# qbxlvnf11/yolo-series

Measured on AMD Instinct MI355X. Metric: images/sec (640×640) + mAP@0.5 parity vs ref; 1/2/4/8 MI355X, higher is better.
Workload: dtype f16; 1 GPU; yolov7 P5 640x640 bs=32/GPU f16: libyv7 forward + GPU NMS (conf 0.25, iou 0.45, max_det 300); global_batch=32, img=640, parallelism=dp1, rccl_world_size=1, weights=seeded synthetic, resident_input_batches=4

## Files before the change

yolo-series_amd/csrc/conv_det.hip:

```cpp
#include <cstdlib>

#include "conv_det.h"
#include "conv_f16_launch.h"

namespace yv7 {

namespace {

template <int HOOK = 0>
__global__ __launch_bounds__(512, 1) void conv_det_pring_kernel(const ConvParams p) {
  constexpr int BM = 64, BN = 256, WM = 2, WN = 4, NW = 8, NTH = 512;
  constexpr int WTM = BM / WM, WTN = BN / WN, TM = WTM / 16, TN = WTN / 16;
  constexpr int RB = BN / 8 / NW;
  constexpr int PER = HOOK == 4 ? 1 : 1 + RB;
  constexpr int STAGE = (BM + BN) * ROWB;
  constexpr int RING = 2 * STAGE;
  constexpr int LDS = RING + det_lds(BM, BN);
  static_assert(LDS <= 160 * 1024, "LDS budget");
  __shared__ __attribute__((aligned(16))) unsigned char smem[LDS];
  unsigned char* es = smem + RING;

  const int tid = threadIdx.x, lane = tid & 63;
  const int wave = __builtin_amdgcn_readfirstlane(tid >> 6);
  const int wm = wave / WN, wn = wave % WN;
// ... 4 lines not shown
  const int ntl = tw.count();
  if (ntl == 0) return;

  const auto xr = make_rsrc(p.x, p.xbytes);
  const auto wr = make_rsrc(p.w, p.wbytes);
  const int lr = lane >> 3;
  const int c = (lane & 7) ^ lr;
  uint32_t b_off[RB];
#pragma unroll
  for (int j = 0; j < RB; ++j) b_off[j] = (uint32_t)((((j * NW + wave) * 8 + lr) * p.kpad + c * 8) * 2);
  const int hw = p.Ho * p.Wo;
  auto a_off = [&](int it) -> uint32_t {
    if (it >= ntl) return OOB;
    const int m = tw.at(it) * BM + wave * 8 + lr;
    if (m >= p.M) return OOB;
    const int b = m / hw, cell = m - b * hw, ho = cell / p.Wo, wo = cell - ho * p.Wo;
    return (uint32_t)((pix_index(b, ho, wo, p.H, p.W) * p.xc + p.xoff + c * 8) * 2);
  };
  int i_it = 0, i_k = 0, i_q = 0;
  uint32_t i_aoff = a_off(0);
  auto issue = [&]() __attribute__((always_inline)) {
    unsigned char* As = smem + (i_q & 1) * STAGE;
    unsigned char* Bs = As + BM * ROWB;
    const bool live = i_it < ntl;
    const uint32_t so = (uint32_t)i_k * BKE * 2;
    dma16(xr, As + wave * 8 * ROWB, i_aoff, so);
    if constexpr (HOOK != 4) {
#pragma unroll
      for (int j = 0; j < RB; ++j) dma16(wr, Bs + (j * NW + wave) * 8 * ROWB, live ? b_off[j] : OOB, so);
    }
// ... 121 lines not shown
  const int g = lane >> 4, li = lane & 15;
  const int m0 = blockIdx.x * BM;
  if (m0 >= p.M) return;
  const int nk = p.kpad / BKE;
  const auto xr = make_rsrc(p.x, p.xbytes);
  const auto wr = make_rsrc(p.w, p.wbytes);
  const int lr = lane >> 3;
  const int c = (lane & 7) ^ lr;
  uint32_t b_off[RB];
#pragma unroll
  for (int j = 0; j < RB; ++j) b_off[j] = (uint32_t)((((j * NW + wave) * 8 + lr) * p.kpad + c * 8) * 2);
  const int hw = p.Ho * p.Wo;
  uint32_t aoff = OOB;
  {
    const int m = m0 + wave * 8 + lr;
    if (m < p.M) {
      const int b = m / hw, cell = m - b * hw, ho = cell / p.Wo, wo = cell - ho * p.Wo;
      aoff = (uint32_t)((pix_index(b, ho, wo, p.H, p.W) * p.xc + p.xoff + c * 8) * 2);
    }
  }
  auto issue = [&](int k, int slot) __attribute__((always_inline)) {
    unsigned char* As = smem + slot * STAGE;
    unsigned char* Bs = As + BM * ROWB;
    const uint32_t so = (uint32_t)k * BKE * 2;
    dma16(xr, As + wave * 8 * ROWB, aoff, so);
#pragma unroll
    for (int j = 0; j < RB; ++j) dma16(wr, Bs + (j * NW + wave) * 8 * ROWB, b_off[j], so);
    asm volatile("" ::: "memory");
  };
  f4 acc[TN][TM];
#pragma unroll
// ... 98 lines not shown
  u4 wreg[TN][NCH];
#pragma unroll
  for (int j = 0; j < TN; ++j) {
    const uint32_t base = (uint32_t)(((2 * wave + j) * NCH) * 1024 + lane * 16);
#pragma unroll
    for (int c = 0; c < NCH; ++c)
      wreg[j][c] = __builtin_bit_cast(u4, __builtin_amdgcn_raw_buffer_load_b128(wr, base, (uint32_t)(c * 1024), 0));
  }
  const int lr = lane >> 3;
  const int c8 = (lane & 7) ^ lr;
  const int hw = p.Ho * p.Wo;
  auto a_off = [&](int it) -> uint32_t {
    if (it >= ntl) return OOB;
    const int m = tw.at(it) * BM + (wave % (BM / 8)) * 8 + lr;
    if (m >= p.M) return OOB;
    const int b = m / hw, cell = m - b * hw, ho = cell / p.Wo, wo = cell - ho * p.Wo;
    return (uint32_t)((pix_index(b, ho, wo, p.H, p.W) * p.xc + p.xoff + c8 * 8) * 2);
  };
  int i_it = 0, i_k = 0, i_slot = 0;
  uint32_t i_aoff = a_off(0);
  auto issue = [&]() __attribute__((always_inline)) {
    if constexpr (HOOK != 1) dma16(xr, smem + i_slot * STAGE + (wave % (BM / 8)) * 8 * ROWB, i_aoff, (uint32_t)i_k * BKE * 2);
    asm volatile("" ::: "memory");
    if (++i_slot == R) i_slot = 0;
    if (++i_k == NK) {
      i_k = 0;
      ++i_it;
      i_aoff = a_off(i_it);
    }
  };
// ... 93 lines not shown
}

bool det_rw_supported(const ConvParams& p) {
  return p.wf && (p.kpad == 256 || p.kpad == 512) && p.wfbytes >= (uint32_t)(256 * p.kpad * 2);
}

}

bool det_pring_supported(const ConvParams& p) {
  const int hw = p.Ho * p.Wo;
  return p.k == 1 && p.s == 1 && p.na == 3 && p.no == 85 && p.cout == 255 && p.raw == nullptr &&
         p.kpad == p.cin && p.cin % BKE == 0 && p.cin >= 2 * BKE && hw % 4 == 0 && p.row_off % 4 == 0 &&
         p.nrows % 4 == 0 && p.xoff % 8 == 0 && p.xc % 8 == 0 && p.H == p.Ho && p.W == p.Wo;
}

hipError_t launch_det_pring(const ConvParams& p, hipStream_t st) {
  const long T = (p.M + 63) / 64, cus = device_cus();
  const long per = (T + cus - 1) / cus;
  const int grid = (int)((T + per - 1) / per);
  static const int rw = env_int("YV7_DET_RW", 1);
  if (rw && (p.variant == 0 || p.variant == 91) && det_rw_supported(p)) {
    if (p.variant == 91) {
      if (p.kpad == 256) YV7_LAUNCH((conv_det_rw_kernel<8, 1>), dim3(grid), dim3(512), 0, st, p);
      else YV7_LAUNCH((conv_det_rw_kernel<16, 1>), dim3(grid), dim3(512), 0, st, p);
      return hipGetLastError();
    }
    static const int rwd = env_int("YV7_DET_RWD", 4);
    static const int bm_env = env_int("YV7_DET_BM", 0);
    const int bm = bm_env ? bm_env : (p.kpad == 512 ? 32 : 64);
    if (bm == 32 && rwd == 4) {
      const long T2 = (p.M + 31) / 32, per2 = (T2 + cus - 1) / cus;
// ... 29 lines not shown
```

yolo-series_amd/csrc/conv_f16_common.h:

```cpp
#pragma once
#include "yv7_kernels.h"

namespace yv7 {

namespace {

constexpr int NT = 256;
constexpr int BKE = 64;
constexpr int ROWB = 128;

__device__ __forceinline__ int swz(int row, int chunk) { return chunk ^ (row & 7); }

struct PixelWalk {
  int b, ho, wo;
  __device__ __forceinline__ PixelWalk(const ConvParams& p, int m) {
    const int hw = p.Ho * p.Wo;
    b = m / hw;
    const int rem = m - b * hw;
    ho = rem / p.Wo;
    wo = rem - ho * p.Wo;
  }
  __device__ __forceinline__ void advance(const ConvParams& p, int step) {
    wo += step;
    while (wo >= p.Wo) {
      wo -= p.Wo;
      if (++ho == p.Ho) { ho = 0; ++b; }
    }
  }
};

__device__ __forceinline__ uint32_t a_origin(const ConvParams& p, int b, int ho, int wo, int chunk) {
  return (uint32_t)((pix_index(b, ho * p.s - p.pad, wo * p.s - p.pad, p.H, p.W) * p.xc + p.xoff + chunk * 8) * 2);
}

template <int BK = BKE>
struct KCursor {
  int ci, rr, ss, tap;
  __device__ __forceinline__ void init(const ConvParams& p, int k) {
    ci = k; rr = ss = tap = 0;
    while (ci >= p.cin) { ci -= p.cin; ++tap; if (++ss == p.k) { ss = 0; ++rr; } }
  }
  __device__ __forceinline__ void advance(const ConvParams& p) {
    ci += BK;
    while (ci >= p.cin) { ci -= p.cin; ++tap; if (++ss == p.k) { ss = 0; ++rr; } }
  }
  __device__ __forceinline__ uint32_t offset(const ConvParams& p) const {
    return (uint32_t)(((rr * (p.W + 2 * BORDER) + ss) * p.xc + ci) * 2);
// ... 84 lines not shown
```

yolo-series_amd/csrc/conv_f16_p8.hip:

```cpp
#include "conv_f16_common.h"
#include "conv_f16_launch.h"

namespace yv7 {

namespace {

template <bool ONE, int ACT, int BM = 256, int BN = 256>
__global__ __launch_bounds__(512, 1) void conv_f16_p8_kernel(const ConvParams p) {
  constexpr int NTH = 512;
  constexpr int AHR = BM / 2, BHR = BN / 2;
  constexpr int AHB = AHR * ROWB, BHB = BHR * ROWB;
  constexpr int BUF = 2 * AHB + 2 * BHB;
  constexpr int AP = AHR / 64, BP = BHR / 64;
  constexpr int VMC = 2 * AP + BP;
  constexpr int WNC = BHR / 32;
  static_assert(AP >= 1 && BP >= 1 && (AHR / 64) * WNC == 8, "8 waves of 64 x 32 per block quadrant");
  constexpr int BIASB = (2 * BUF + 4096 + 16 <= 163840) ? 4096 : 0;
  __shared__ __attribute__((aligned(16))) unsigned char smem[2 * BUF + BIASB];
  float* bias_l = reinterpret_cast<float*>(smem + 2 * BUF);

  const int tid = threadIdx.x, lane = tid & 63;
  const int wave = __builtin_amdgcn_readfirstlane(tid >> 6);
  const int wm = wave / WNC, wn = wave % WNC;
  const int grp = wave >> 2;
// ... 11 lines not shown
  auto tile_at = [&](int it) { return tw.at(it); };

  const auto xr = make_rsrc(p.x, p.xbytes);
  const auto wr = make_rsrc(p.w, p.wbytes);
  const auto yr = make_rsrc(p.y, 0x7fffffffu);
  if constexpr (BIASB != 0)
    for (int i = tid; i < p.cout; i += NTH) bias_l[i] = p.bias[i];

  int a_it = 0, a_kt = 0, b_it = 0, b_kt = 0;
  uint32_t a_off[2][AP], b_off[2][BP], a_so = 0;
  KWalk sa, sb;
  auto stage_a = [&](int h, int par) {
    if (h == 0) {
      if (a_kt == 0) {
        const int t = tile_at(a_it);
        PixelWalk pw(p, (t / nN) * BM + wave * 8 + lr);
#pragma unroll
        for (int q = 0; q < 2 * AP; ++q) {
          if (q) pw.advance(p, 64);
          a_off[q / AP][q % AP] = a_origin(p, pw.b, pw.ho, pw.wo, c);
        }
        sa.init();
      }
      a_so = ONE ? (uint32_t)a_kt * BKE * 2 : sa.a_offset(p);
      if (!ONE) sa.advance(p);
    }
    unsigned char* d = smem + par * BUF + h * AHB;
#pragma unroll
    for (int j = 0; j < AP; ++j) dma16(xr, d + (j * 8 + wave) * 8 * ROWB, a_off[h][j], a_so);
    if (h == 1) {
      if (++a_kt == nk) { a_kt = 0; ++a_it; }
    }
  };
  uint32_t b_so = 0;
  auto stage_b = [&](int h, int par) {
    if (h == 1) {
// ... 29 lines not shown
        const int col = cn0 + hb * BHR + wn * 32 + j * 16 + g * 4;
        f4 bv;
#pragma unroll
        for (int e = 0; e < 4; ++e)
          bv[e] = col + e < p.cout ? (BIASB ? bias_l[col + e] : p.bias[col + e]) : 0.0f;
#pragma unroll
        for (int ha = 0; ha < 2; ++ha)
#pragma unroll
          for (int i = 0; i < 4; ++i) acc[hb][j][ha][i] = bv;
      }
  };
  const uint32_t lane_ch = (uint32_t)(16 * (g & 1) + 8 * (g >> 1));
  auto epilogue = [&]() {
#pragma unroll
    for (int ha = 0; ha < 2; ++ha) {
      PixelWalk pw(p, cm0 + ha * AHR + wm * 64 + li);
#pragma unroll
      for (int i = 0; i < 4; ++i) {
        if (i) pw.advance(p, 16);
        const int m = cm0 + ha * AHR + wm * 64 + i * 16 + li;
        const uint32_t yo = (uint32_t)((pix_index(pw.b, pw.ho, pw.wo, p.Ho, p.Wo) * p.yc + p.yoff) * 2);
#pragma unroll
        for (int hb = 0; hb < 2; ++hb) {
          typedef _Float16 h4 __attribute__((ext_vector_type(4)));
          typedef uint32_t u2 __attribute__((ext_vector_type(2)));
          h4 va, vb;
          const f4 a0 = acc[hb][0][ha][i], a1 = acc[hb][1][ha][i];
#pragma unroll
          for (int e = 0; e < 4; ++e) {
            va[e] = (_Float16)act_t<ACT>(a0[e]);
            vb[e] = (_Float16)act_t<ACT>(a1[e]);
          }
          const u2 a = __builtin_bit_cast(u2, va), b = __builtin_bit_cast(u2, vb);
          const auto s0 = __builtin_amdgcn_permlane16_swap(a[0], b[0], false, false);
          const auto s1 = __builtin_amdgcn_permlane16_swap(a[1], b[1], false, false);
          const u4 v = {s0[0], s1[0], s0[1], s1[1]};
// ... 65 lines not shown
    if (n2) stage_a(0, P);
    mfma_q(0, 1);
    read_a(bk + AHB);
    if (n2) stage_b(1, P);
    mfma_q(1, 1);
    read_b(bk + 2 * AHB);
    if (n2) {
      stage_a(1, P);
      asm volatile("s_waitcnt vmcnt(%0)" ::"n"(VMC) : "memory");
    } else {
      asm volatile("s_waitcnt vmcnt(0)" ::: "memory");
    }
    mfma_q(1, 0);
  };
  auto fresh_a = [&](int t) __attribute__((always_inline)) {
    PixelWalk pw(p, (t / nN) * BM + wave * 8 + lr);
#pragma unroll
    for (int q = 0; q < 2 * AP; ++q) {
      if (q) pw.advance(p, 64);
      a_off[q / AP][q % AP] = a_origin(p, pw.b, pw.ho, pw.wo, c);
    }
  };
  auto fresh_b = [&](int t) __attribute__((always_inline)) {
    const int n0 = t % nN * BN;
#pragma unroll
    for (int q = 0; q < 2 * BP; ++q)
      b_off[q / BP][q % BP] = (uint32_t)(((n0 + (q / BP) * BHR + ((q % BP) * 8 + wave) * 8 + lr) * p.kpad + c * 8) * 2);
  };
  auto dma_a = [&](int h, int par, uint32_t so) __attribute__((always_inline)) {
    unsigned char* d = smem + par * BUF + h * AHB;
#pragma unroll
    for (int j = 0; j < AP; ++j) dma16(xr, d + (j * 8 + wave) * 8 * ROWB, a_off[h][j], so);
  };
  auto dma_b = [&](int h, int par, uint32_t so) __attribute__((always_inline)) {
    unsigned char* d = smem + par * BUF + 2 * AHB + h * BHB;
#pragma unroll
// ... 99 lines not shown
  const int total = ntl * nk;
  if (total == 0) return;

  const auto xr = make_rsrc(p.x, p.xbytes);
  const auto wr = make_rsrc(p.w, p.wbytes);
  const auto yr = make_rsrc(p.y, 0x7fffffffu);
  for (int i = tid; i < p.cout; i += NTH) bias_l[i] = p.bias[i];

  int s_it = 0, s_kt = 0;
  uint32_t a_off[2][2], b_off[2], a_so = 0, b_so = 0;
  KWalk su;
  auto stage = [&](int h, int par) {
    if (h == 0) {
      if (s_kt == 0) {
        const int t = tw.at(s_it);
        PixelWalk pw(p, (t / nN) * BM + wave * 8 + lr);
#pragma unroll
        for (int q = 0; q < 4; ++q) {
          if (q) pw.advance(p, 64);
          a_off[q >> 1][q & 1] = a_origin(p, pw.b, pw.ho, pw.wo, c);
        }
        const int n0 = t % nN * BN;
#pragma unroll
        for (int q = 0; q < 2; ++q) b_off[q] = (uint32_t)(((n0 + q * 64 + wave * 8 + lr) * p.kpad + c * 8) * 2);
        su.init();
      }
      a_so = ONE ? (uint32_t)s_kt * BKE * 2 : su.a_offset(p);
      b_so = ONE ? (uint32_t)s_kt * BKE * 2 : su.b_offset(p);
      if (!ONE) su.advance(p);
    }
    unsigned char* d = smem + par * BUF;
#pragma unroll
    for (int j = 0; j < 2; ++j) dma16(xr, d + h * AH + (j * 8 + wave) * 8 * ROWB, a_off[h][j], a_so);
    dma16(wr, d + 2 * AH + h * BH + wave * 8 * ROWB, b_off[h], b_so);
    if (h == 1) {
      if (++s_kt == nk) { s_kt = 0; ++s_it; }
// ... 10 lines not shown
    for (int j = 0; j < 4; ++j) {
      const int col = cn0 + wn * 64 + j * 16 + g * 4;
      f4 bv;
#pragma unroll
      for (int e = 0; e < 4; ++e) bv[e] = col + e < p.cout ? bias_l[col + e] : 0.0f;
#pragma unroll
      for (int h = 0; h < 2; ++h)
#pragma unroll
        for (int i = 0; i < 2; ++i) acc[h][j][i] = bv;
    }
  };
  const uint32_t lane_ch = (uint32_t)(16 * (g & 1) + 8 * (g >> 1));
  auto epilogue = [&]() {
#pragma unroll
    for (int h = 0; h < 2; ++h) {
      PixelWalk pw(p, cm0 + h * 128 + wm * 32 + li);
#pragma unroll
      for (int i = 0; i < 2; ++i) {
        if (i) pw.advance(p, 16);
        const int m = cm0 + h * 128 + wm * 32 + i * 16 + li;
        const uint32_t yo = (uint32_t)((pix_index(pw.b, pw.ho, pw.wo, p.Ho, p.Wo) * p.yc + p.yoff) * 2);
#pragma unroll
        for (int mp = 0; mp < 2; ++mp) {
          typedef _Float16 h4 __attribute__((ext_vector_type(4)));
          typedef uint32_t u2 __attribute__((ext_vector_type(2)));
          h4 va, vb;
#pragma unroll
          for (int e = 0; e < 4; ++e) {
            va[e] = (_Float16)act_t<ACT>(acc[h][2 * mp][i][e]);
            vb[e] = (_Float16)act_t<ACT>(acc[h][2 * mp + 1][i][e]);
          }
          const u2 a = __builtin_bit_cast(u2, va), b = __builtin_bit_cast(u2, vb);
          const auto s0 = __builtin_amdgcn_permlane16_swap(a[0], b[0], false, false);
          const auto s1 = __builtin_amdgcn_permlane16_swap(a[1], b[1], false, false);
          const u4 v = {s0[0], s1[0], s0[1], s1[1]};
          const int n = cn0 + wn * 64 + mp * 32 + (int)lane_ch;
// ... 82 lines not shown
    for (int k = 0; k < total; ++k) {
      ktile(k % 3, k + 2 < total);
      if (++ckt == nk) {
        epilogue();
        ckt = 0;
        if (++ci < ntl) init_tile(ci);
      }
    }
  }
  if (grp == 0) __builtin_amdgcn_s_barrier();
  asm volatile("s_waitcnt vmcnt(0)" ::: "memory");
}

}

hipError_t launch_p8(const ConvParams& p, int cfg, hipStream_t st) {
  const bool one = p.k == 1 && p.s == 1 && p.pad == 0;
  if (cfg != P8_256x256 && cfg != P8_256x128) return hipErrorInvalidValue;
  if (p.cout > 1024 || p.cout % 8 || p.yoff % 8 || p.yc % 8 || (!one && p.cin % BKE)) return hipErrorInvalidValue;
  const int bn = cfg == P8_256x256 ? 256 : 128;
  const long T = (long)((p.M + 255) / 256) * ((p.cout + bn - 1) / bn);
  const int cus = device_cus();
  const int grid = (int)(T < (long)cus ? T : (long)cus);
  return launch_with_act(p.act, [&](auto A) {
    constexpr int ACT = decltype(A)::value;
    if (cfg == P8_256x256) {
      if (one) YV7_LAUNCH((conv_f16_p8_kernel<true, ACT>), dim3(grid), dim3(512), 0, st, p);
      else YV7_LAUNCH((conv_f16_p8_kernel<false, ACT>), dim3(grid), dim3(512), 0, st, p);
    } else {
      if (one) YV7_LAUNCH((conv_f16_p8n_kernel<true, ACT>), dim3(grid), dim3(512), 0, st, p);
      else YV7_LAUNCH((conv_f16_p8n_kernel<false, ACT>), dim3(grid), dim3(512), 0, st, p);
// ... 7 lines not shown
```

yolo-series_amd/csrc/conv_f16_pring.hip:

```cpp
#include "conv_f16_common.h"
#include "conv_f16_launch.h"

namespace yv7 {

namespace {

template <int BM, int BN, int WM, int WN, int STAGES, bool ONE, int ACT, int BK, int WS = 0, int HOOK = 0>
__global__ __launch_bounds__(64 * WM * WN, (STAGES * (BM + BN) * BK * 2 <= 48 * 1024 && WM * WN == 4) ? 3 : (STAGES * (BM + BN) * BK * 2 <= 76 * 1024) ? 2 : 1) void conv_f16_pring_kernel(
    const ConvParams p) {
  constexpr int NW = WM * WN, NTH = 64 * NW;
  constexpr int WTM = BM / WM, WTN = BN / WN;
  constexpr int TM = WTM / 16, TN = WTN / 16;
  constexpr int RB_ = BK * 2;
  constexpr int CPR = RB_ / 16;
  constexpr int RPI = 64 / CPR;
  constexpr int RA = BM / RPI / NW, RB = BN / RPI / NW;
  static_assert(RA * RPI * NW == BM && RB * RPI * NW == BN, "tile rows must split into DMA groups per wave");
  static_assert(TN % 2 == 0, "the epilogue pairs 16-channel groups");
  static_assert(STAGES >= 2 && STAGES <= 4, "counted waits cover up to two stages in flight");
  static_assert(WS == 0 || ONE, "weight-stationary form: 1x1 convs only");
  constexpr int PER = RA + (WS ? 0 : RB);
  constexpr int NST = TM * TN / 2;
  constexpr int STAGE = (BM + (WS ? 0 : BN)) * RB_;
  constexpr int WREG = WS ? BN * WS * RB_ : 0;
// ... 41 lines not shown
    for (int q = wave; q < nk * GPS; q += NW) {
      const int ks = q / GPS, rg = q - ks * GPS;
      dma16(wr, wl + (ks * BN + rg * RPI) * RB_, (uint32_t)(((nb * BN + rg * RPI + lr) * p.kpad + c * 8) * 2),
            (uint32_t)ks * BK * 2);
    }
  }

  AWalk<ONE, RA, BK> aw;
  uint32_t b_off[RB];
  int ig = 0, it = 0, ikt = 0;
  auto issue_next = [&]() __attribute__((always_inline)) {
    if (ikt == 0) {
      const int t = tw.at(it);
      const int m0 = tile_m0(t), n0 = tile_n0(t);
      aw.init(p, c, 0);
      PixelWalk pw(p, m0 + wave * RPI + lr);
#pragma unroll
      for (int j = 0; j < RA; ++j) {
        if (j) pw.advance(p, NW * RPI);
        aw.off[j] = a_origin(p, pw.b, pw.ho, pw.wo, c);
      }
#pragma unroll
      for (int j = 0; j < RB; ++j) b_off[j] = (uint32_t)(((n0 + (j * NW + wave) * RPI + lr) * p.kpad + c * 8) * 2);
    }
    const int slot = ig % STAGES;
    unsigned char* As = smem + slot * STAGE;
    unsigned char* Bs = As + BM * RB_;
    if constexpr (HOOK != 298) {
      aw.step(p, ikt, [&](int j, uint32_t vo, uint32_t so) { dma16(xr, As + (j * NW + wave) * RPI * RB_, vo, so); });
      if constexpr (WS == 0) {
#pragma unroll
        for (int j = 0; j < RB; ++j) dma16(wr, Bs + (j * NW + wave) * RPI * RB_, b_off[j], (uint32_t)ikt * BK * 2);
      }
    }
    ++ig;
    if (++ikt == nk) { ikt = 0; ++it; }
// ... 20 lines not shown
#pragma unroll
    for (int j = 0; j < TN; ++j)
#pragma unroll
      for (int ii = 0; ii < TM; ++ii) asm volatile("" : "+v"(acc[j][ii]));
    if constexpr (HOOK == 296 || HOOK == 297) {
      float sink = 0.0f;
#pragma unroll
      for (int ii = 0; ii < TM; ++ii)
#pragma unroll
        for (int j = 0; j < TN; ++j)
#pragma unroll
          for (int e = 0; e < 4; ++e) sink += HOOK == 297 ? acc[j][ii][e] : act_t<ACT>(acc[j][ii][e]);
      if (sink == 12345.0f) __builtin_amdgcn_raw_buffer_store_b32(__builtin_bit_cast(uint32_t, sink), yr, 0, 0, 0);
      return;
    }
    PixelWalk pw(p, cm0 + wm * WTM + li);
#pragma unroll
    for (int ii = 0; ii < TM; ++ii) {
      if (ii) pw.advance(p, 16);
      const int m = cm0 + wm * WTM + ii * 16 + li;
      const uint32_t yo = (uint32_t)((pix_index(pw.b, pw.ho, pw.wo, p.Ho, p.Wo) * p.yc + p.yoff) * 2);
#pragma unroll
      for (int mp = 0; mp < TN / 2; ++mp) {
        typedef _Float16 h4 __attribute__((ext_vector_type(4)));
        typedef uint32_t u2 __attribute__((ext_vector_type(2)));
        h4 va, vb;
#pragma unroll
        for (int e = 0; e < 4; ++e) {
          va[e] = (_Float16)act_t<ACT>(acc[2 * mp][ii][e]);
          vb[e] = (_Float16)act_t<ACT>(acc[2 * mp + 1][ii][e]);
        }
        const u2 a = __builtin_bit_cast(u2, va), b = __builtin_bit_cast(u2, vb);
        const auto s0 = __builtin_amdgcn_permlane16_swap(a[0], b[0], false, false);
        const auto s1 = __builtin_amdgcn_permlane16_swap(a[1], b[1], false, false);
        const u4 v = {s0[0], s1[0], s0[1], s1[1]};
        const int n = cn0 + wn * WTN + mp * 32 + (int)lane_ch;
// ... 68 lines not shown
    kstep(gs, std::integral_constant<int, 0>{});
    kstep(gs + 1, std::integral_constant<int, 1>{});
    if constexpr (STAGES > 2) kstep(gs + 2, std::integral_constant<int, (STAGES > 2 ? 2 : 0)>{});
    if constexpr (STAGES > 3) kstep(gs + 3, std::integral_constant<int, (STAGES > 3 ? 3 : 0)>{});
  }
  if constexpr (UNROLL) {
    if (gs < nsteps) kstep(gs++, std::integral_constant<int, 0>{});
    if (STAGES > 2 && gs < nsteps) kstep(gs++, std::integral_constant<int, 1>{});
    if (STAGES > 3 && gs < nsteps) kstep(gs++, std::integral_constant<int, (STAGES > 3 ? 2 : 0)>{});
  }
  asm volatile("s_waitcnt vmcnt(0)" ::: "memory");
}

}

hipError_t launch_pring(const ConvParams& p, int row, hipStream_t st) {
  const bool one = p.k == 1 && p.s == 1 && p.pad == 0;
  return launch_with_row<NPRING>(row, [&](auto I) {
    constexpr PringRow r = pring_rows[decltype(I)::value];
    constexpr int BM = r.bm, BN = r.bn;
    const dim3 block(64 * r.wm * r.wn);
    if constexpr (r.kind == PR_HOOK) {
      const long T = (long)((p.M + 255) / 256) * ((p.cout + 255) / 256);
      const int grid = (int)(T < (long)device_cus() ? T : (long)device_cus());
      if (one) YV7_LAUNCH((conv_f16_pring_kernel<BM, BN, r.wm, r.wn, r.stages, true, 1, 64, 0, r.hook>), dim3(grid), block, 0, st, p);
      else YV7_LAUNCH((conv_f16_pring_kernel<BM, BN, r.wm, r.wn, r.stages, false, 1, 64, 0, r.hook>), dim3(grid), block, 0, st, p);
      return hipGetLastError();
    } else if constexpr (r.kind == PR_WSN) {
      const int nN = (p.cout + BN - 1) / BN;
      if (nN < 2 || p.cout % 8 || p.yoff % 8 || p.yc % 8 || p.kpad > r.ws * 64 || p.k != 1 || p.s != 1 || p.pad)
        return hipErrorInvalidValue;
// ... 33 lines not shown
```

yolo-series_amd/csrc/conv_f16_ring.hip:

```cpp
#include "conv_det.h"
#include "conv_f16_launch.h"

namespace yv7 {

namespace {

__device__ __forceinline__ u4 hmax4(u4 a, u4 b, u4 c, u4 d) {
  const h8 m = __builtin_elementwise_max(__builtin_elementwise_max(__builtin_bit_cast(h8, a), __builtin_bit_cast(h8, b)),
                                         __builtin_elementwise_max(__builtin_bit_cast(h8, c), __builtin_bit_cast(h8, d)));
  return __builtin_bit_cast(u4, m);
}

template <int TM>
__device__ __forceinline__ void res_rows(const ConvParams& p, int m_first, uint32_t (&ro)[TM]) {
#pragma unroll
  for (int i = 0; i < TM; ++i) {
    const int m = m_first + i * 16;
    ro[i] = OOB;
    if (m < p.M) {
      PixelWalk pw(p, m);
      ro[i] = (uint32_t)((pix_index(pw.b, pw.ho, pw.wo, p.Ho, p.Wo) * p.rc + p.roff) * 2);
    }
  }
}
typedef _Float16 h4r __attribute__((ext_vector_type(4)));
__device__ __forceinline__ h4r res_load(__amdgpu_buffer_rsrc_t rr, uint32_t row, int n, int cout) {
  const uint32_t vo = (row != OOB && n < cout) ? row + (uint32_t)n * 2 : OOB;
  return __builtin_bit_cast(h4r, __builtin_amdgcn_raw_buffer_load_b64(rr, vo, 0, 0));
}

template <int BM, int BN, int WM, bool ONE, bool DET, int PF, bool POOL, bool RES>
__device__ __forceinline__ void conv_f16_body(const ConvParams& p) {
  constexpr int WN = 4 / WM;
  constexpr int WTM = BM / WM, WTN = BN / WN;
  constexpr int TM = WTM / 16, TN = WTN / 16;
  constexpr int RA = BM / 32;
  constexpr int RB = (BN + 31) / 32;
// ... 11 lines not shown

  const int nwg = gridDim.x, bid = blockIdx.x;
  const int q = nwg >> 3, r = nwg & 7, xcd = bid & 7, loc = bid >> 3;
  const int wgid = (xcd < r ? xcd * (q + 1) : r * (q + 1) + (xcd - r) * q) + loc;
  const int nN = (p.cout + BN - 1) / BN;
  const int m0 = (wgid / nN) * BM, n0 = (wgid % nN) * BN;

  const auto xr = make_rsrc(p.x, p.xbytes);
  const auto wr = make_rsrc(p.w, p.wbytes);

  const int c = tid & 7;
  const int r0 = tid >> 3;

  AWalk<ONE, RA> aw;
  aw.init(p, c);
  {
    PixelWalk pw(p, m0 + r0);
#pragma unroll
    for (int j = 0; j < RA; ++j) {
      if (j) pw.advance(p, 32);
      aw.off[j] = a_origin(p, pw.b, pw.ho, pw.wo, c);
    }
  }
  uint32_t b_off[RB];
#pragma unroll
  for (int j = 0; j < RB; ++j) b_off[j] = (uint32_t)(((n0 + r0 + 32 * j) * p.kpad + c * 8) * 2);

  const int nk = p.kpad / BKE;
  const uint32_t pdx = (uint32_t)p.xc * 2, pdy = (uint32_t)(p.W + 2 * BORDER) * p.xc * 2;
  auto gload = [&](int kt, u4 (&ra)[RA], u4 (&rb)[RB]) {
    aw.step(p, kt, [&](int j, uint32_t vo, uint32_t so) {
      if constexpr (POOL) {
        const u4 a = __builtin_bit_cast(u4, __builtin_amdgcn_raw_buffer_load_b128(xr, vo, so, 0));
        const u4 b = __builtin_bit_cast(u4, __builtin_amdgcn_raw_buffer_load_b128(xr, vo + pdx, so, 0));
        const u4 c2 = __builtin_bit_cast(u4, __builtin_amdgcn_raw_buffer_load_b128(xr, vo + pdy, so, 0));
        const u4 d = __builtin_bit_cast(u4, __builtin_amdgcn_raw_buffer_load_b128(xr, vo + pdy + pdx, so, 0));
        ra[j] = hmax4(a, b, c2, d);
      } else {
// ... 80 lines not shown
      if (kt + 3 < nk) gload(kt + 3, ra2, rb2);
      compute(1);
      if (kt + 2 < nk) lstore(0, ra, rb);
      __syncthreads();
    }
  }

  if constexpr (DET) {
    det_epilogue<BM, BN, NT>(p, smem, acc, m0, wm, wn, g, li, tid);
    return;
  }

  uint32_t* yrow = reinterpret_cast<uint32_t*>(smem + BM * CPITCH);
  if (tid < BM) {
    const int m = m0 + tid;
    uint32_t v = ~0u;
    if (m < p.M) {
      PixelWalk pw(p, m);
      v = (uint32_t)(pix_index(pw.b, pw.ho, pw.wo, p.Ho, p.Wo) * p.yc + p.yoff);
    }
    yrow[tid] = v;
  }
  unsigned char* Cs = smem;
  [[maybe_unused]] uint32_t rrow[TM];
  [[maybe_unused]] const auto rr = make_rsrc(RES ? p.res : p.zero, RES ? p.rbytes : 0u);
  if constexpr (RES) res_rows<TM>(p, m0 + wm * WTM + li, rrow);
  with_act(p.act, [&](auto actc) {
    constexpr int ACT = decltype(actc)::value;
#pragma unroll
    for (int j = 0; j < TN; ++j) {
      const int col = wn * WTN + j * 16 + g * 4;
      [[maybe_unused]] h4r rv[TM];
      if constexpr (RES) {
#pragma unroll
        for (int i = 0; i < TM; ++i) rv[i] = res_load(rr, rrow[i], n0 + col, p.cout);
      }
// ... 107 lines not shown
  const int S = (!DET && p.ksplit > 1) ? p.ksplit : 1;
  const int tile = wgid / S, ks = wgid - tile * S;
  const int nN = (p.cout + BN - 1) / BN;
  const int m0 = (tile / nN) * BM, n0 = (tile % nN) * BN;
  const int nk_all = p.kpad / BKE;
  const int kb = ks * nk_all / S, ke = (ks + 1) * nk_all / S;

  const auto xr = make_rsrc(p.x, p.xbytes);
  const auto wr = make_rsrc(p.w, p.wbytes);

  const int lr = lane >> 3;
  const int c = (lane & 7) ^ lr;

  AWalk<ONE, RA> aw;
  aw.init(p, c, kb);
  {
    PixelWalk pw(p, m0 + wave * 8 + lr);
#pragma unroll
    for (int j = 0; j < RA; ++j) {
      if (j) pw.advance(p, NW * 8);
      aw.off[j] = a_origin(p, pw.b, pw.ho, pw.wo, c);
    }
  }
  uint32_t b_off[RB];
#pragma unroll
  for (int j = 0; j < RB; ++j) b_off[j] = (uint32_t)(((n0 + (j * NW + wave) * 8 + lr) * p.kpad + c * 8) * 2);

  const int nk = ke - kb;
  auto issue = [&](int kt, int slot) {
    unsigned char* As = smem + slot * STAGE;
    unsigned char* Bs = As + BM * ROWB;
    aw.step(p, kb + kt, [&](int j, uint32_t vo, uint32_t so) { dma16(xr, As + (j * NW + wave) * 8 * ROWB, vo, so); });
#pragma unroll
    for (int j = 0; j < RB; ++j) dma16(wr, Bs + (j * NW + wave) * 8 * ROWB, b_off[j], (uint32_t)(kb + kt) * BKE * 2);
  };

  f4 acc[TN][TM];
#pragma unroll
// ... 47 lines not shown
    }
    if (++slot == STAGES) slot = 0;
  }
  asm volatile("s_waitcnt vmcnt(0) lgkmcnt(0)" ::: "memory");
  __syncthreads();

  if (S > 1 && !splitk_reduce<NTH, TN, TM>(p, smem, acc, tile, ks, S, tid)) return;

  if constexpr (DET) {
    det_epilogue<BM, BN, NTH>(p, smem, acc, m0, wm, wn, g, li, tid);
    return;
  }
  uint32_t* yrow = reinterpret_cast<uint32_t*>(smem + BM * CPITCH);
  for (int t = tid; t < BM; t += NTH) {
    const int m = m0 + t;
    uint32_t v = ~0u;
    if (m < p.M) {
      PixelWalk pw(p, m);
      v = (uint32_t)(pix_index(pw.b, pw.ho, pw.wo, p.Ho, p.Wo) * p.yc + p.yoff);
    }
    yrow[t] = v;
  }
  unsigned char* Cs = smem;
  [[maybe_unused]] uint32_t rrow[TM];
  [[maybe_unused]] const auto rr = make_rsrc(RES ? p.res : p.zero, RES ? p.rbytes : 0u);
  if constexpr (RES) res_rows<TM>(p, m0 + wm * WTM + li, rrow);
  with_act(p.act, [&](auto actc) {
    constexpr int ACT = decltype(actc)::value;
#pragma unroll
    for (int j = 0; j < TN; ++j) {
      const int col = wn * WTN + j * 16 + g * 4;
      [[maybe_unused]] h4r rv[TM];
      if constexpr (RES) {
#pragma unroll
        for (int i = 0; i < TM; ++i) rv[i] = res_load(rr, rrow[i], n0 + col, p.cout);
      }
// ... 31 lines not shown
}
template <int BM, int BN, int WM, bool ONE>
__global__ __launch_bounds__(NT, 2) void conv_f16_res_kernel(const ConvParams p) {
  conv_f16_body<BM, BN, WM, ONE, false, 1, false, true>(p);
}
template <int BM, int BN, int WM, int WN, int STAGES, bool ONE, bool DET = false>
__global__ __launch_bounds__(64 * WM * WN, (STAGES * (BM + BN) * 128 <= 80 * 1024) ? 2 : 1) void conv_f16_ring_kernel(const ConvParams p) {
  conv_f16_ring_body<BM, BN, WM, WN, STAGES, ONE, DET, false>(p);
}
template <int BM, int BN, int WM, int WN, int STAGES, bool ONE>
__global__ __launch_bounds__(64 * WM * WN, (STAGES * (BM + BN) * 128 <= 80 * 1024) ? 2 : 1) void conv_f16_ring_res_kernel(const ConvParams p) {
  conv_f16_ring_body<BM, BN, WM, WN, STAGES, ONE, false, true>(p);
}

template <int BM, int BN, int WM, bool ONE, bool DET, int PF, bool POOL, bool RES>
hipError_t launch_t(const ConvParams& p, hipStream_t st) {
  const int nM = (p.M + BM - 1) / BM, nN = (p.cout + BN - 1) / BN;
  if (DET && p.cout > BN) return hipErrorInvalidValue;
  if constexpr (RES) {
    static_assert(!DET && !POOL && PF == 1, "the residual rows are plain tiles");
    if (!p.res) return hipErrorInvalidValue;
    YV7_LAUNCH((conv_f16_res_kernel<BM, BN, WM, ONE>), dim3(nM * nN), dim3(NT), 0, st, p);
  } else {
    if (p.res) return hipErrorInvalidValue;
    YV7_LAUNCH((conv_f16_kernel<BM, BN, WM, ONE, DET, PF, POOL>), dim3(nM * nN), dim3(NT), 0, st, p);
  }
  return hipGetLastError();
}

template <int BM, int BN, int WM, int WN, int STAGES, bool ONE, bool DET, bool RES>
hipError_t launch_r(const ConvParams& p0, int S, hipStream_t st) {
  ConvParams p = p0;
  if (DET && p.cout > BN) return hipErrorInvalidValue;
  const long tiles = (long)((p.M + BM - 1) / BM) * ((p.cout + BN - 1) / BN);
  unsigned nblk = (unsigned)tiles;
  if (S >= 1) {
    p.ksplit = S;
    if (S > 1 && (!p.part || !p.cnt || p.part_bytes < (size_t)tiles * S * BM * BN * 4 || p.cnt_n < tiles))
      return hipErrorInvalidValue;
    nblk = (unsigned)(tiles * S);
  }
  if constexpr (RES) {
    static_assert(!DET, "the residual rows are plain rings");
    if (!p.res) return hipErrorInvalidValue;
    YV7_LAUNCH((conv_f16_ring_res_kernel<BM, BN, WM, WN, STAGES, ONE>), dim3(nblk), dim3(64 * WM * WN), 0, st, p);
  } else {
    if (p.res) return hipErrorInvalidValue;
// ... 29 lines not shown
```

yolo-series_amd/csrc/conv_lr.hip:

```cpp
#include "yv7_kernels.h"

namespace yv7 {

namespace {

constexpr int FI = 4, FC = 4;
constexpr int CK = 32;

__host__ __device__ constexpr int swz(int img) { return (0x1320 >> (4 * img)) & 3; }

template <int S> __host__ __device__ constexpr int patch_cols() { return S == 1 ? FC + 2 : 2 * FC + 1; }
template <int S> __host__ __device__ constexpr int col_slot(int c) { return S == 1 ? c : ((c & 1) ? 5 + (c >> 1) : (c >> 1)); }

template <int WM, int WN, int TM, int S>
struct LrGeo {
  static constexpr int NT = 64 * WM * WN;
  static constexpr int TH = TM * WM, PR = S * TH + 3 - S, PC = patch_cols<S>();
  static constexpr int PPX = FI * PR * PC;
  static constexpr int PB = PPX * 64;
};

struct LrRow { int wm, wn, tn, tm, pd, s, pf; };
constexpr LrRow lr_rows[] = {
    {1, 4, 2, 5, 3, 1, 1}, {1, 4, 1, 5, 3, 1, 1},  {1, 4, 2, 4, 3, 1, 1},  {1, 4, 1, 4, 3, 1, 1},
// ... 12 lines not shown
  constexpr int PPX = G::PPX;
  constexpr int PB = G::PB;
  constexpr int NPL = (PPX * 4 + NT - 1) / NT;
  constexpr int NPH = 3 * NCH;
  constexpr int NWB = PD + 1;

  const int tid = threadIdx.x, lane = tid & 63;
  const int wave = __builtin_amdgcn_readfirstlane(tid >> 6);
  const int wm = wave / WN, wn = wave % WN;
  const int g = lane >> 4, li = lane & 15;

  const auto xr = make_rsrc(p.x, p.xbytes);
  const auto wr = make_rsrc(p.wf, p.wfbytes);
  const auto yr = make_rsrc(p.y, 0x7fffffffu);

  uint32_t po[NPL], pd[NPL];
#pragma unroll
  for (int k = 0; k < NPL; ++k) {
    const int q = tid + k * NT;
    const int px = q >> 2, qq = q & 3;
    if (px < PPX) {
      const int img = px / (PR * PC), r2 = px - img * (PR * PC);
      const int row = r2 / PC, col = r2 - row * PC;
      po[k] = (uint32_t)((pix_index(b0 + img, S * y0 - 1 + row, S * x0 - 1 + col, p.H, p.W) * p.xc + p.xoff + qq * 8) * 2);
      pd[k] = (uint32_t)(((img * PR + row) * PC + col_slot<S>(col)) * 64 + ((qq ^ swz(img)) * 16));
    } else {
      po[k] = OOB;
      pd[k] = 0xffffffffu;
    }
  }
  u4 pr[PF][NPL];
  auto load_patch = [&](int c) __attribute__((always_inline)) {
#pragma unroll
// ... 68 lines not shown
#pragma unroll
    for (int s = 0; s < 3; ++s) {
      const int ph = c * 3 + s;
      if (ph + PD < NPH) load_w(ph + PD, wreg[(ph + PD) % NWB]);
      u4 xa[NXA];
      read_xa(c, s, xa);
      mfmas(ph, xa);
    }
    if (c + 1 < NCH) {
      store_patch(c + 1);
      if (c + 1 + PF < NCH) load_patch(c + 1 + PF);
      __syncthreads();
    }
  }

#pragma unroll
  for (int i = 0; i < TM; ++i) {
    const bool live = b0 + img < p.B;
    const uint32_t yo =
        live ? (uint32_t)((pix_index(b0 + img, y0 + wm * TM + i, x0 + (li & 3), p.Ho, p.Wo) * p.yc + p.yoff) * 2)
             : 0x80000000u;
    typedef _Float16 h4 __attribute__((ext_vector_type(4)));
    typedef uint32_t u2 __attribute__((ext_vector_type(2)));
    if constexpr (TN % 2 == 0) {
      const uint32_t lane_ch = (uint32_t)(16 * (g & 1) + 8 * (g >> 1));
#pragma unroll
      for (int mp = 0; mp < TN / 2; ++mp) {
        h4 va, vb;
#pragma unroll
        for (int e = 0; e < 4; ++e) {
          va[e] = (_Float16)act_t<ACT>(acc[2 * mp][i][e]);
          vb[e] = (_Float16)act_t<ACT>(acc[2 * mp + 1][i][e]);
        }
        const u2 a = __builtin_bit_cast(u2, va), b = __builtin_bit_cast(u2, vb);
        const auto s0 = __builtin_amdgcn_permlane16_swap(a[0], b[0], false, false);
        const auto s1 = __builtin_amdgcn_permlane16_swap(a[1], b[1], false, false);
// ... 310 lines not shown
```

yolo-series_amd/csrc/yv7_kernels.h:

```cpp
#pragma once
#include <hip/hip_ext.h>
#include <hip/hip_runtime.h>
#include <stdint.h>

#include <cstdlib>
#include <type_traits>
#include <utility>

namespace yv7 {

struct OpEvents {
  hipEvent_t start = nullptr, stop = nullptr;
  int launches = 0;
};
inline OpEvents& op_events() {
  static thread_local OpEvents e;
  return e;
}
struct LaunchRec {
  bool dry = false;
  int n = 0;
  const void* fn[4] = {nullptr, nullptr, nullptr, nullptr};
};
inline LaunchRec& launch_rec() {
// ... 129 lines not shown
  float stride, anchor[8];
  int variant;
  float* part;
  int* cnt;
  size_t part_bytes;
  int cnt_n;
  int ksplit;
  int pool;
  const void* wf;
  uint32_t wfbytes;
  const void* res;
  uint32_t rbytes;
  int rc, roff;
  Div24 d0, d1;
};

struct Conv1x1Pooled {
  const void* w;
  const float* bias;
  void* y;
  int yc, yoff, cout, act;
};
bool conv1x1_rs_supported(const ConvParams& p, const Conv1x1Pooled* q);
hipError_t launch_conv1x1_rs(const ConvParams& p, const Conv1x1Pooled* q, hipStream_t st);

size_t conv_splitk_part_bytes(const ConvParams& p);
int conv_splitk_tiles(const ConvParams& p);

struct F8ConvParams {
  const void* x8;
// ... 97 lines not shown
```

Measured before the change: 7869 images/sec.

## Use precomputed 24-bit reciprocal division for pixel address computation in conv kernels

Replaces the integer division and modulo chains (PixelWalk, pix_index) used to turn a flat output row index into bordered NHWC addresses with 24-bit magic-multiply division (Div24) precomputed on the host and passed in ConvParams. This applies across the det, p8, pring, ring and lr conv kernels. The lr kernel also gets a TRIM path that walks patch and output offsets incrementally instead of recomputing them per element. The aim is to cut scalar and vector integer ALU work in address setup and epilogues. The fast path is gated on size bounds, can be disabled with an environment variable, and adds more code paths with a risk of overflow edge cases.

```diff
diff --git a/yolo-series_amd/csrc/conv_det.hip b/yolo-series_amd/csrc/conv_det.hip
--- a/yolo-series_amd/csrc/conv_det.hip
+++ b/yolo-series_amd/csrc/conv_det.hip
@@ -42,6 +42,7 @@
     if (it >= ntl) return OOB;
     const int m = tw.at(it) * BM + wave * 8 + lr;
     if (m >= p.M) return OOB;
+    if (addr32(p)) return a_origin32<true>(p, m, c);
     const int b = m / hw, cell = m - b * hw, ho = cell / p.Wo, wo = cell - ho * p.Wo;
     return (uint32_t)((pix_index(b, ho, wo, p.H, p.W) * p.xc + p.xoff + c * 8) * 2);
   };
@@ -193,7 +194,9 @@
   uint32_t aoff = OOB;
   {
     const int m = m0 + wave * 8 + lr;
-    if (m < p.M) {
+    if (m < p.M && addr32(p)) {
+      aoff = a_origin32<true>(p, m, c);
+    } else if (m < p.M) {
       const int b = m / hw, cell = m - b * hw, ho = cell / p.Wo, wo = cell - ho * p.Wo;
       aoff = (uint32_t)((pix_index(b, ho, wo, p.H, p.W) * p.xc + p.xoff + c * 8) * 2);
     }
@@ -322,6 +325,7 @@
     if (it >= ntl) return OOB;
     const int m = tw.at(it) * BM + (wave % (BM / 8)) * 8 + lr;
     if (m >= p.M) return OOB;
+    if (addr32(p)) return a_origin32<true>(p, m, c8);
     const int b = m / hw, cell = m - b * hw, ho = cell / p.Wo, wo = cell - ho * p.Wo;
     return (uint32_t)((pix_index(b, ho, wo, p.H, p.W) * p.xc + p.xoff + c8 * 8) * 2);
   };
@@ -445,7 +449,8 @@
          p.nrows % 4 == 0 && p.xoff % 8 == 0 && p.xc % 8 == 0 && p.H == p.Ho && p.W == p.Wo;
 }
 
-hipError_t launch_det_pring(const ConvParams& p, hipStream_t st) {
+hipError_t launch_det_pring(const ConvParams& p0, hipStream_t st) {
+  const ConvParams p = fill_addr32(p0);
   const long T = (p.M + 63) / 64, cus = device_cus();
   const long per = (T + cus - 1) / cus;
   const int grid = (int)((T + per - 1) / per);
diff --git a/yolo-series_amd/csrc/conv_f16_common.h b/yolo-series_amd/csrc/conv_f16_common.h
--- a/yolo-series_amd/csrc/conv_f16_common.h
+++ b/yolo-series_amd/csrc/conv_f16_common.h
@@ -31,6 +31,59 @@
 
 __device__ __forceinline__ uint32_t a_origin(const ConvParams& p, int b, int ho, int wo, int chunk) {
   return (uint32_t)((pix_index(b, ho * p.s - p.pad, wo * p.s - p.pad, p.H, p.W) * p.xc + p.xoff + chunk * 8) * 2);
+}
+
+__device__ __forceinline__ bool addr32(const ConvParams& p) { return p.d0.mul != 0; }
+
+template <bool ONE>
+__device__ __forceinline__ uint32_t a_origin32(const ConvParams& p, int m, int chunk) {
+  const uint32_t lane = (uint32_t)(p.xoff + chunk * 8) * 2;
+  if constexpr (ONE) {
+    return pix_index32(m, p.W, p.d0, p.d1) * (uint32_t)(p.xc * 2) + lane;
+  } else {
+    const int R = div24(m, p.d0), b = div24(R, p.d1);
+    const int ho = R - b * p.Ho, wo = m - R * p.Wo;
+    const int pitch = p.W + 2 * BORDER;
+    const int idx = b * ((p.H + 2 * BORDER) * pitch) + ho * (p.s * pitch) + wo * p.s + (BORDER - p.pad) * (pitch + 1);
+    return (uint32_t)idx * (uint32_t)(p.xc * 2) + lane;
+  }
+}
+
+template <bool ONE, int N, typename F>
+__device__ __forceinline__ void a_origins(const ConvParams& p, int m0, int step, int chunk, F&& set) {
+  if (addr32(p)) {
+#pragma unroll
+    for (int j = 0; j < N; ++j) set(j, a_origin32<ONE>(p, m0 + j * step, chunk));
+  } else {
+    PixelWalk pw(p, m0);
+#pragma unroll
+    for (int j = 0; j < N; ++j) {
+      if (j) pw.advance(p, step);
+      set(j, a_origin(p, pw.b, pw.ho, pw.wo, chunk));
+    }
+  }
+}
+
+__device__ __forceinline__ uint32_t out_elem(const ConvParams& p, int m, int pitch, int off) {
+  if (addr32(p)) return pix_index32(m, p.Wo, p.d0, p.d1) * (uint32_t)pitch + (uint32_t)off;
+  PixelWalk pw(p, m);
+  return (uint32_t)(pix_index(pw.b, pw.ho, pw.wo, p.Ho, p.Wo) * pitch + off);
+}
+
+template <int N, typename F>
+__device__ __forceinline__ void y_offsets(const ConvParams& p, int m0, int step, F&& set) {
+  if (addr32(p)) {
+#pragma unroll
+    for (int j = 0; j < N; ++j)
+      set(j, pix_index32(m0 + j * step, p.Wo, p.d0, p.d1) * (uint32_t)(p.yc * 2) + (uint32_t)(p.yoff * 2));
+  } else {
+    PixelWalk pw(p, m0);
+#pragma unroll
+    for (int j = 0; j < N; ++j) {
+      if (j) pw.advance(p, step);
+      set(j, (uint32_t)((pix_index(pw.b, pw.ho, pw.wo, p.Ho, p.Wo) * p.yc + p.yoff) * 2));
+    }
+  }
 }
 
 template <int BK = BKE>
diff --git a/yolo-series_amd/csrc/conv_f16_p8.hip b/yolo-series_amd/csrc/conv_f16_p8.hip
--- a/yolo-series_amd/csrc/conv_f16_p8.hip
+++ b/yolo-series_amd/csrc/conv_f16_p8.hip
@@ -49,12 +49,8 @@
     if (h == 0) {
       if (a_kt == 0) {
         const int t = tile_at(a_it);
-        PixelWalk pw(p, (t / nN) * BM + wave * 8 + lr);
-#pragma unroll
-        for (int q = 0; q < 2 * AP; ++q) {
-          if (q) pw.advance(p, 64);
-          a_off[q / AP][q % AP] = a_origin(p, pw.b, pw.ho, pw.wo, c);
-        }
+        a_origins<ONE, 2 * AP>(p, (t / nN) * BM + wave * 8 + lr, 64, c,
+                               [&](int q, uint32_t o) { a_off[q / AP][q % AP] = o; });
         sa.init();
       }
       a_so = ONE ? (uint32_t)a_kt * BKE * 2 : sa.a_offset(p);
@@ -114,12 +110,12 @@
   auto epilogue = [&]() {
 #pragma unroll
     for (int ha = 0; ha < 2; ++ha) {
-      PixelWalk pw(p, cm0 + ha * AHR + wm * 64 + li);
+      uint32_t yrow[4];
+      y_offsets<4>(p, cm0 + ha * AHR + wm * 64 + li, 16, [&](int i, uint32_t o) { yrow[i] = o; });
 #pragma unroll
       for (int i = 0; i < 4; ++i) {
-        if (i) pw.advance(p, 16);
         const int m = cm0 + ha * AHR + wm * 64 + i * 16 + li;
-        const uint32_t yo = (uint32_t)((pix_index(pw.b, pw.ho, pw.wo, p.Ho, p.Wo) * p.yc + p.yoff) * 2);
+        const uint32_t yo = yrow[i];
 #pragma unroll
         for (int hb = 0; hb < 2; ++hb) {
           typedef _Float16 h4 __attribute__((ext_vector_type(4)));
@@ -215,12 +211,7 @@
     mfma_q(1, 0);
   };
   auto fresh_a = [&](int t) __attribute__((always_inline)) {
-    PixelWalk pw(p, (t / nN) * BM + wave * 8 + lr);
-#pragma unroll
-    for (int q = 0; q < 2 * AP; ++q) {
-      if (q) pw.advance(p, 64);
-      a_off[q / AP][q % AP] = a_origin(p, pw.b, pw.ho, pw.wo, c);
-    }
+    a_origins<ONE, 2 * AP>(p, (t / nN) * BM + wave * 8 + lr, 64, c, [&](int q, uint32_t o) { a_off[q / AP][q % AP] = o; });
   };
   auto fresh_b = [&](int t) __attribute__((always_inline)) {
     const int n0 = t % nN * BN;
@@ -350,12 +341,7 @@
     if (h == 0) {
       if (s_kt == 0) {
         const int t = tw.at(s_it);
-        PixelWalk pw(p, (t / nN) * BM + wave * 8 + lr);
-#pragma unroll
-        for (int q = 0; q < 4; ++q) {
-          if (q) pw.advance(p, 64);
-          a_off[q >> 1][q & 1] = a_origin(p, pw.b, pw.ho, pw.wo, c);
-        }
+        a_origins<ONE, 4>(p, (t / nN) * BM + wave * 8 + lr, 64, c, [&](int q, uint32_t o) { a_off[q >> 1][q & 1] = o; });
         const int n0 = t % nN * BN;
 #pragma unroll
         for (int q = 0; q < 2; ++q) b_off[q] = (uint32_t)(((n0 + q * 64 + wave * 8 + lr) * p.kpad + c * 8) * 2);
@@ -396,12 +382,12 @@
   auto epilogue = [&]() {
 #pragma unroll
     for (int h = 0; h < 2; ++h) {
-      PixelWalk pw(p, cm0 + h * 128 + wm * 32 + li);
+      uint32_t yrow[2];
+      y_offsets<2>(p, cm0 + h * 128 + wm * 32 + li, 16, [&](int i, uint32_t o) { yrow[i] = o; });
 #pragma unroll
       for (int i = 0; i < 2; ++i) {
-        if (i) pw.advance(p, 16);
         const int m = cm0 + h * 128 + wm * 32 + i * 16 + li;
-        const uint32_t yo = (uint32_t)((pix_index(pw.b, pw.ho, pw.wo, p.Ho, p.Wo) * p.yc + p.yoff) * 2);
+        const uint32_t yo = yrow[i];
 #pragma unroll
         for (int mp = 0; mp < 2; ++mp) {
           typedef _Float16 h4 __attribute__((ext_vector_type(4)));
@@ -514,7 +500,8 @@
 
 }
 
-hipError_t launch_p8(const ConvParams& p, int cfg, hipStream_t st) {
+hipError_t launch_p8(const ConvParams& p0, int cfg, hipStream_t st) {
+  const ConvParams p = fill_addr32(p0);
   const bool one = p.k == 1 && p.s == 1 && p.pad == 0;
   if (cfg != P8_256x256 && cfg != P8_256x128) return hipErrorInvalidValue;
   if (p.cout > 1024 || p.cout % 8 || p.yoff % 8 || p.yc % 8 || (!one && p.cin % BKE)) return hipErrorInvalidValue;
diff --git a/yolo-series_amd/csrc/conv_f16_pring.hip b/yolo-series_amd/csrc/conv_f16_pring.hip
--- a/yolo-series_amd/csrc/conv_f16_pring.hip
+++ b/yolo-series_amd/csrc/conv_f16_pring.hip
@@ -79,12 +79,7 @@
       const int t = tw.at(it);
       const int m0 = tile_m0(t), n0 = tile_n0(t);
       aw.init(p, c, 0);
-      PixelWalk pw(p, m0 + wave * RPI + lr);
-#pragma unroll
-      for (int j = 0; j < RA; ++j) {
-        if (j) pw.advance(p, NW * RPI);
-        aw.off[j] = a_origin(p, pw.b, pw.ho, pw.wo, c);
-      }
+      a_origins<ONE, RA>(p, m0 + wave * RPI + lr, NW * RPI, c, [&](int j, uint32_t o) { aw.off[j] = o; });
 #pragma unroll
       for (int j = 0; j < RB; ++j) b_off[j] = (uint32_t)(((n0 + (j * NW + wave) * RPI + lr) * p.kpad + c * 8) * 2);
     }
@@ -135,12 +130,12 @@
       if (sink == 12345.0f) __builtin_amdgcn_raw_buffer_store_b32(__builtin_bit_cast(uint32_t, sink), yr, 0, 0, 0);
       return;
     }
-    PixelWalk pw(p, cm0 + wm * WTM + li);
+    uint32_t yrow[TM];
+    y_offsets<TM>(p, cm0 + wm * WTM + li, 16, [&](int ii, uint32_t o) { yrow[ii] = o; });
 #pragma unroll
     for (int ii = 0; ii < TM; ++ii) {
-      if (ii) pw.advance(p, 16);
       const int m = cm0 + wm * WTM + ii * 16 + li;
-      const uint32_t yo = (uint32_t)((pix_index(pw.b, pw.ho, pw.wo, p.Ho, p.Wo) * p.yc + p.yoff) * 2);
+      const uint32_t yo = yrow[ii];
 #pragma unroll
       for (int mp = 0; mp < TN / 2; ++mp) {
         typedef _Float16 h4 __attribute__((ext_vector_type(4)));
@@ -239,7 +234,8 @@
 
 }
 
-hipError_t launch_pring(const ConvParams& p, int row, hipStream_t st) {
+hipError_t launch_pring(const ConvParams& p0, int row, hipStream_t st) {
+  const ConvParams p = fill_addr32(p0);
   const bool one = p.k == 1 && p.s == 1 && p.pad == 0;
   return launch_with_row<NPRING>(row, [&](auto I) {
     constexpr PringRow r = pring_rows[decltype(I)::value];
diff --git a/yolo-series_amd/csrc/conv_f16_ring.hip b/yolo-series_amd/csrc/conv_f16_ring.hip
--- a/yolo-series_amd/csrc/conv_f16_ring.hip
+++ b/yolo-series_amd/csrc/conv_f16_ring.hip
@@ -17,10 +17,7 @@
   for (int i = 0; i < TM; ++i) {
     const int m = m_first + i * 16;
     ro[i] = OOB;
-    if (m < p.M) {
-      PixelWalk pw(p, m);
-      ro[i] = (uint32_t)((pix_index(pw.b, pw.ho, pw.wo, p.Ho, p.Wo) * p.rc + p.roff) * 2);
-    }
+    if (m < p.M) ro[i] = out_elem(p, m, p.rc, p.roff) * 2;
   }
 }
 typedef _Float16 h4r __attribute__((ext_vector_type(4)));
@@ -62,14 +59,7 @@
 
   AWalk<ONE, RA> aw;
   aw.init(p, c);
-  {
-    PixelWalk pw(p, m0 + r0);
-#pragma unroll
-    for (int j = 0; j < RA; ++j) {
-      if (j) pw.advance(p, 32);
-      aw.off[j] = a_origin(p, pw.b, pw.ho, pw.wo, c);
-    }
-  }
+  a_origins<ONE, RA>(p, m0 + r0, 32, c, [&](int j, uint32_t o) { aw.off[j] = o; });
   uint32_t b_off[RB];
 #pragma unroll
   for (int j = 0; j < RB; ++j) b_off[j] = (uint32_t)(((n0 + r0 + 32 * j) * p.kpad + c * 8) * 2);
@@ -180,12 +170,7 @@
   uint32_t* yrow = reinterpret_cast<uint32_t*>(smem + BM * CPITCH);
   if (tid < BM) {
     const int m = m0 + tid;
-    uint32_t v = ~0u;
-    if (m < p.M) {
-      PixelWalk pw(p, m);
-      v = (uint32_t)(pix_index(pw.b, pw.ho, pw.wo, p.Ho, p.Wo) * p.yc + p.yoff);
-    }
-    yrow[tid] = v;
+    yrow[tid] = m < p.M ? out_elem(p, m, p.yc, p.yoff) : ~0u;
   }
   unsigned char* Cs = smem;
   [[maybe_unused]] uint32_t rrow[TM];
@@ -323,14 +308,7 @@
 
   AWalk<ONE, RA> aw;
   aw.init(p, c, kb);
-  {
-    PixelWalk pw(p, m0 + wave * 8 + lr);
-#pragma unroll
-    for (int j = 0; j < RA; ++j) {
-      if (j) pw.advance(p, NW * 8);
-      aw.off[j] = a_origin(p, pw.b, pw.ho, pw.wo, c);
-    }
-  }
+  a_origins<ONE, RA>(p, m0 + wave * 8 + lr, NW * 8, c, [&](int j, uint32_t o) { aw.off[j] = o; });
   uint32_t b_off[RB];
 #pragma unroll
   for (int j = 0; j < RB; ++j) b_off[j] = (uint32_t)(((n0 + (j * NW + wave) * 8 + lr) * p.kpad + c * 8) * 2);
@@ -408,12 +386,7 @@
   uint32_t* yrow = reinterpret_cast<uint32_t*>(smem + BM * CPITCH);
   for (int t = tid; t < BM; t += NTH) {
     const int m = m0 + t;
-    uint32_t v = ~0u;
-    if (m < p.M) {
-      PixelWalk pw(p, m);
-      v = (uint32_t)(pix_index(pw.b, pw.ho, pw.wo, p.Ho, p.Wo) * p.yc + p.yoff);
-    }
-    yrow[t] = v;
+    yrow[t] = m < p.M ? out_elem(p, m, p.yc, p.yoff) : ~0u;
   }
   unsigned char* Cs = smem;
   [[maybe_unused]] uint32_t rrow[TM];
@@ -475,7 +448,8 @@
 }
 
 template <int BM, int BN, int WM, bool ONE, bool DET, int PF, bool POOL, bool RES>
-hipError_t launch_t(const ConvParams& p, hipStream_t st) {
+hipError_t launch_t(const ConvParams& p0, hipStream_t st) {
+  const ConvParams p = fill_addr32(p0);
   const int nM = (p.M + BM - 1) / BM, nN = (p.cout + BN - 1) / BN;
   if (DET && p.cout > BN) return hipErrorInvalidValue;
   if constexpr (RES) {
@@ -491,7 +465,7 @@
 
 template <int BM, int BN, int WM, int WN, int STAGES, bool ONE, bool DET, bool RES>
 hipError_t launch_r(const ConvParams& p0, int S, hipStream_t st) {
-  ConvParams p = p0;
+  ConvParams p = fill_addr32(p0);
   if (DET && p.cout > BN) return hipErrorInvalidValue;
   const long tiles = (long)((p.M + BM - 1) / BM) * ((p.cout + BN - 1) / BN);
   unsigned nblk = (unsigned)tiles;
diff --git a/yolo-series_amd/csrc/conv_lr.hip b/yolo-series_amd/csrc/conv_lr.hip
--- a/yolo-series_amd/csrc/conv_lr.hip
+++ b/yolo-series_amd/csrc/conv_lr.hip
@@ -50,9 +50,38 @@
   const auto wr = make_rsrc(p.wf, p.wfbytes);
   const auto yr = make_rsrc(p.y, 0x7fffffffu);
 
+  constexpr bool TRIM = TM <= 5 && CPL == 0 && CPS == 0 && !(TN == 2 && TM == 5 && NCH == 2 && ACT == 2 && S == 1);
   uint32_t po[NPL], pd[NPL];
-#pragma unroll
-  for (int k = 0; k < NPL; ++k) {
+  if constexpr (TRIM) {
+    constexpr int STEP = NT / 4, IMG = PR * PC;
+    constexpr int DI = STEP / IMG, DR = STEP % IMG / PC, DC = STEP % PC;
+    static_assert(NT % 4 == 0, "a thread's pieces are whole pixels apart");
+    const int qq = tid & 3;
+    int px = tid >> 2;
+    int img = px / IMG, row = (px - img * IMG) / PC, col = px - img * IMG - row * PC;
+    const uint32_t pitch = (uint32_t)(p.W + 2 * BORDER), ipitch = (uint32_t)(p.H + 2 * BORDER) * pitch;
+    const uint32_t xc2 = (uint32_t)p.xc * 2;
+    const uint32_t base = ((uint32_t)(b0 * (p.H + 2 * BORDER) + S * y0) * pitch + (uint32_t)(S * x0)) * xc2;
+    const uint32_t lch = (uint32_t)(p.xoff + qq * 8) * 2;
+#pragma unroll
+    for (int k = 0; k < NPL; ++k) {
+      if (px < PPX) {
+        po[k] = base + ((uint32_t)img * ipitch + (uint32_t)row * pitch + (uint32_t)col) * xc2 + lch;
+        pd[k] = (uint32_t)(((img * PR + row) * PC + col_slot<S>(col)) * 64 + ((qq ^ swz(img)) * 16));
+      } else {
+        po[k] = OOB;
+        pd[k] = 0xffffffffu;
+      }
+      px += STEP;
+      col += DC;
+      if (col >= PC) { col -= PC; ++row; }
+      row += DR;
+      if (row >= PR) { row -= PR; ++img; }
+      img += DI;
+    }
+  }
+#pragma unroll
+  for (int k = 0; k < (TRIM ? 0 : NPL); ++k) {
     const int q = tid + k * NT;
     const int px = q >> 2, qq = q & 3;
     if (px < PPX) {
@@ -151,12 +180,22 @@
     }
   }
 
+  [[maybe_unused]] uint32_t yo0 = 0, ystep = 0;
+  if constexpr (TRIM) {
+    const uint32_t ypitch = (uint32_t)(p.Wo + 2 * BORDER);
+    const uint32_t pix = (uint32_t)((b0 + img) * (p.Ho + 2 * BORDER) + y0 + wm * TM + BORDER) * ypitch + (uint32_t)(x0 + (li & 3) + BORDER);
+    yo0 = (pix * (uint32_t)p.yc + (uint32_t)p.yoff) * 2;
+    ystep = ypitch * (uint32_t)p.yc * 2;
+  }
 #pragma unroll
   for (int i = 0; i < TM; ++i) {
     const bool live = b0 + img < p.B;
-    const uint32_t yo =
-        live ? (uint32_t)((pix_index(b0 + img, y0 + wm * TM + i, x0 + (li & 3), p.Ho, p.Wo) * p.yc + p.yoff) * 2)
-             : 0x80000000u;
+    uint32_t yo;
+    if constexpr (TRIM)
+      yo = yo0 + (uint32_t)i * ystep;
+    else
+      yo = live ? (uint32_t)((pix_index(b0 + img, y0 + wm * TM + i, x0 + (li & 3), p.Ho, p.Wo) * p.yc + p.yoff) * 2)
+                : 0x80000000u;
     typedef _Float16 h4 __attribute__((ext_vector_type(4)));
     typedef uint32_t u2 __attribute__((ext_vector_type(2)));
     if constexpr (TN % 2 == 0) {
diff --git a/yolo-series_amd/csrc/yv7_kernels.h b/yolo-series_amd/csrc/yv7_kernels.h
--- a/yolo-series_amd/csrc/yv7_kernels.h
+++ b/yolo-series_amd/csrc/yv7_kernels.h
@@ -167,6 +167,25 @@
   int rc, roff;
   Div24 d0, d1;
 };
+
+__device__ __forceinline__ uint32_t pix_index32(int m, int W, Div24 dw, Div24 dh) {
+  const int R = div24(m, dw), b = div24(R, dh);
+  return (uint32_t)(m + 2 * BORDER * R + (2 * b + 1) * BORDER * (W + 2 * BORDER) + BORDER);
+}
+
+constexpr int ADDR32_TILE = 512;
+inline bool addr32_ok(const ConvParams& p) {
+  return p.M > 0 && p.M <= (1 << 24) - ADDR32_TILE && p.Wo >= 1 && p.Ho >= 1 &&
+         bordered_pixels(p.B, p.Ho, p.Wo) * (size_t)p.yc * 2 < ((size_t)1 << 32);
+}
+inline ConvParams fill_addr32(const ConvParams& p0) {
+  ConvParams p = p0;
+  static const bool off = env_int("YV7_NO_ADDR32", 0) != 0;
+  const bool ok = addr32_ok(p) && !off;
+  p.d0 = ok ? make_div24(p.Wo) : Div24{0u, 0u};
+  p.d1 = ok ? make_div24(p.Ho) : Div24{0u, 0u};
+  return p;
+}
 
 struct Conv1x1Pooled {
   const void* w;
```

Result: no change. 7906 images/sec (median of 6 runs) (+0.5%).
